# LuletterSoul/RP-Style-Transfer

Measured on AMD Instinct MI355X. Metric: stylized images/sec at 512×512, 1/2/4/8 MI355X; % HBM roofline, higher is better.
Workload: dtype fp32

## Files before the change

rp-style-transfer_amd/csrc/rpst_wino4.hip:

```cpp
#include "rpst_conv.h"
#include "rpst_wct.h"

#include <type_traits>

namespace rpst {

typedef __attribute__((address_space(3))) void* lds_ptr_t;

constexpr int kW4CK = 8;
#ifndef RPST_W4DBG
#define RPST_W4DBG 0
#endif
constexpr int kW4HW = 0, kW4HP = 2;
constexpr int kW4Ahead = 2, kW4Ahead2 = 3;
constexpr int kW4BM = 32;
constexpr int kW4TH = 16, kW4TW = 64;
constexpr int kW4PH = kW4TH + 2;
constexpr int kW4PS = 68;
constexpr int kW4CS = 1280;
constexpr int kW4DMA = 20;
constexpr int kW4DMA4 = 5;
constexpr int kW4WCH = 36 * kW4BM * kW4CK;
constexpr int kW4SPATCH = 4 * kW4CS;
constexpr int kW4SW = kW4WCH / 2;
// ... 127 lines not shown
  const float* btab;
  float2* statp;
};

__device__ __forceinline__ void bt6(float& d0, float& d1, float& d2, float& d3, float& d4,
                                    float& d5) {
  const float A = fmaf(-4.f, d2, d4), B = fmaf(-4.f, d1, d3);
  const float C = d4 - d2, E = d3 - d1;
  const float t0 = fmaf(4.f, d0, fmaf(-5.f, d2, d4));
  const float t5 = fmaf(4.f, d1, fmaf(-5.f, d3, d5));
  d0 = t0;
  d1 = A + B;
  d2 = A - B;
  d3 = fmaf(2.f, E, C);
  d4 = fmaf(-2.f, E, C);
  d5 = t5;
}

template <int NR, int INOP, bool STATS, bool BTAB, bool RELU>
__global__ __launch_bounds__(W4Geo<NR>::NTH, W4Geo<NR>::LAUNCH_WPE) void wino4_mfma_kernel(ConvArgs a) {
  using Geo = W4Geo<NR>;
  constexpr int S = Geo::STG, NW = Geo::NW, NH = Geo::NH;
  constexpr int DBG = RPST_W4DBG;
  static_assert(RawN<INOP>::R == 1, "one raw load per patch element");
  __shared__ __attribute__((aligned(16))) float smem0[Geo::STAGE];
  __shared__ __attribute__((aligned(16))) float smem1[Geo::STAGE];
  __shared__ __attribute__((aligned(16))) float smem2[S > 2 ? Geo::STAGE : 4];
  __shared__ __attribute__((aligned(16))) float smem3[S > 3 ? Geo::STAGE : 4];
  __shared__ __attribute__((aligned(16))) float dummy[256];

  int bid = (int)blockIdx.x;
  const int cog = bid % a.cosplit;
  bid /= a.cosplit;
  const int nct = a.co_tiles / a.cosplit;
  const int ct0 = cog * nct;
  int tx, ty, n;
  w4_tile(bid, a.tiles_x, a.tiles_y, tx, ty, n);
  const int nch = a.nchunks, K4 = 2 * nch, G = nct * K4;
  const int y0 = ty * Geo::TH, x0 = tx * kW4TW;

  const int tid = threadIdx.x;
  const int lane = tid & 63, wave = __builtin_amdgcn_readfirstlane(tid >> 6);
  const int k = lane >> 4, tn = lane & 15;
  const int wr = wave % NR, ph = wave / NR;

  const bool pooled = INOP == RPST_IN_UPSAMPLE2;
  const unsigned in_plane = pooled ? (unsigned)(a.Hs * a.Ws) : (unsigned)(a.H * a.W);
  const unsigned oob = a.Cin * in_plane * 4u;
  const float* in_img = conv_in_img(a, n, (int64_t)a.Cin * in_plane);
  const unsigned wbytes = (unsigned)(a.co_tiles * nch * kW4WCH) * 4u;
  const float* w_img = a.wpk + (int64_t)n * a.wstride;


  const int chl = wave / NH, hf = wave % NH;
  const bool zp = a.pad == RPST_PAD_ZERO;
  const int rs = pooled ? a.Ws : a.W;
  constexpr bool kAff = INOP == RPST_IN_ADAIN;
  constexpr int kSlow = Geo::SLOW, kWide = Geo::WIDE;
  unsigned poff[kSlow];
  unsigned pvalid = 0;
  const bool wide = !pooled && x0 >= 1 && x0 + kW4TW < a.W;
  {
    if (wide) {
#pragma unroll
      for (int i = 0; i < kWide; ++i) {
        const int p = kWide * hf + i;
        const int f = 64 * p + lane, row = min(f / 17, Geo::PH - 1), j = f - (f / 17) * 17;
        int y = y0 - 1 + row;
        const bool ok = p < Geo::DMA4 && f < Geo::PH * 17 && resolve_bf(y, a.H, zp);
        poff[i] = ok ? ((unsigned)(y * rs) + (unsigned)(x0 - 1 + 4 * j)) * 4u : oob;
        pvalid |= ok ? (1u << i) : 0u;
      }
    } else {
#pragma unroll
      for (int i = 0; i < kSlow; ++i) {
        const int f = 64 * (kSlow * hf + i) + lane;
        const int row = min(f / kW4PS, Geo::PH - 1), col = f - (f / kW4PS) * kW4PS;
        int y = y0 - 1 + row, x = x0 - 1 + col;
        const bool oky = resolve_bf(y, a.H, zp), okx = resolve_bf(x, a.W, zp);
        const bool ok = col < kW4TW + 2 && oky && okx;
        poff[i] = ok ? ((unsigned)((pooled ? y >> 1 : y) * rs) + (unsigned)(pooled ? x >> 1 : x)) * 4u
                     : oob;
        pvalid |= ok ? (1u << i) : 0u;
      }
    }
  }
  __shared__ float aparm[kAff ? 3 * kW4AffC : 1];
  if constexpr (kAff) {
    for (int c = tid; c < a.Cin; c += Geo::NTH) {
      const AdainP p = adain_params(a.aux, n, c, a);
      aparm[c] = p.mc;
      aparm[kW4AffC + c] = p.scale;
      aparm[2 * kW4AffC + c] = p.ms;
    }
    __syncthreads();
  }
  floatx4 acc[18][2];
#pragma unroll
  for (int x = 0; x < 18; ++x) acc[x][0] = acc[x][1] = floatx4{0.f, 0.f, 0.f, 0.f};

  auto issue_w = [&](int g, bool live, float* st) {
    if (!(DBG & 2)) {
      constexpr int WC = Geo::WPI - 1, REST = 18 - WC * NW;
      static_assert(REST > 0 && REST <= NW, "one remainder piece per wave at the most");
      const int wv = launder(wave);
      const int sw = ((ct0 * K4 + g) * kW4SW + wv * (WC * 256)) * 4;
      const auto r = rsrc_or_zero(w_img, wbytes, live);
      float* t = st + Geo::SPATCH + wv * (WC * 256);
      static_assert(WC == 2 || WC == 4, "the contiguous pieces below");
      __builtin_amdgcn_raw_ptr_buffer_load_lds(r, (lds_ptr_t)t, 16, lane * 16, sw, 0, 0);
      __builtin_amdgcn_raw_ptr_buffer_load_lds(r, (lds_ptr_t)t, 16, lane * 16, sw, 1024, 0);
      if constexpr (WC == 4) {
        __builtin_amdgcn_raw_ptr_buffer_load_lds(r, (lds_ptr_t)t, 16, lane * 16, sw, 2048, 0);
        __builtin_amdgcn_raw_ptr_buffer_load_lds(r, (lds_ptr_t)t, 16, lane * 16, sw, 3072, 0);
      }
      const bool real = wv < REST;
      __builtin_amdgcn_raw_ptr_buffer_load_lds(
          rsrc_or_zero(w_img, wbytes, live && real),
          (lds_ptr_t)(real ? st + Geo::SPATCH + (WC * NW + wv) * 256 : dummy), 16, lane * 16,
          sw + (WC * NW - (WC - 1) * wv) * 1024, 0, 0);
    }
  };
  auto issue_p = [&](int ks, bool live, float* st) {
    {
      if (DBG & 1) return;
      const int wv = launder(wave);
      const int c = 4 * ks + wv / NH;
      const bool ok = live && c < a.Cin;
      const auto r = rsrc_or_zero(in_img, oob, ok);
      const int so = ok ? (int)((unsigned)c * in_plane * 4u) : 0;
      float* xs = st + (wv / NH) * Geo::CS;
      if (wide) {
#pragma unroll
        for (int i = 0; i < kWide; ++i) {
          const int p = kWide * (wv % NH) + i;
          __builtin_amdgcn_raw_ptr_buffer_load_lds(
              r, (lds_ptr_t)(p < Geo::DMA4 ? xs + 256 * p : dummy), 16, (int)poff[i], so, 0, 0);
        }
      } else {
#pragma unroll
        for (int i = 0; i < kSlow; ++i)
          __builtin_amdgcn_raw_ptr_buffer_load_lds(r, (lds_ptr_t)(xs + 64 * (kSlow * (wv % NH) + i)),
                                                   4, (int)poff[i], so, 0, 0);
      }
    }
  };
  [[maybe_unused]] auto issue = [&](int g, int ks, bool live, float* st) {
    issue_w(g, live, st);
    issue_p(ks, live, st);
  };
  auto fix_own = [&](int g, float* st) {
    if constexpr (kAff) {
      if (DBG & 4) return;
      const int ks = g % K4, ch = 4 * ks + chl;
      const bool chok = ch < a.Cin;
      const int cc = chok ? ch : 0;
      const float mc = aparm[cc], sc = aparm[kW4AffC + cc], ms = aparm[2 * kW4AffC + cc];
      float* xs = st + chl * Geo::CS;
      if (wide) {
#pragma unroll
        for (int i = 0; i < kWide; ++i) {
          const int p = kWide * hf + i;
          if (p < Geo::DMA4) {
            float4* e = reinterpret_cast<float4*>(xs + 4 * (64 * p + lane));
            const bool ok = chok && ((pvalid >> i) & 1u);
            const float4 v = *e;
            *e = make_float4(ok ? fmaf(v.x - mc, sc, ms) : 0.f, ok ? fmaf(v.y - mc, sc, ms) : 0.f,
                             ok ? fmaf(v.z - mc, sc, ms) : 0.f, ok ? fmaf(v.w - mc, sc, ms) : 0.f);
          }
        }
      } else {
#pragma unroll
        for (int i = 0; i < kSlow; ++i) {
          float* e = xs + 64 * (kSlow * hf + i) + lane;
          const bool ok = chok && ((pvalid >> i) & 1u);
          *e = ok ? fmaf(*e - mc, sc, ms) : 0.f;
        }
      }
    }
  };


  auto load_rows = [&](const float* pbuf, float (&d)[5][6]) {
    const float* pr = pbuf + k * Geo::CS + (4 * wr + ph) * kW4PS + 4 * tn;
#pragma unroll
    for (int r = 0; r < 5; ++r) {
      floatx4 u = *reinterpret_cast<const floatx4*>(pr + r * kW4PS);
      floatx4 v = *reinterpret_cast<const floatx4*>(pr + r * kW4PS + 4);
      asm("" : "+v"(u), "+v"(v));
      d[r][0] = u[0];
      d[r][1] = u[1];
      d[r][2] = u[2];
      d[r][3] = u[3];
      d[r][4] = v[0];
      d[r][5] = v[1];
    }
  };
  auto compute = [&](const float* pbuf, float (&d)[5][6], auto&& hw, auto&& hp) {
    {
      const float* wq = pbuf + Geo::SPATCH + ph * 9 * 256 + lane * 4;
      float4 w4[9];
      constexpr int kA = NR == 4 ? kW4Ahead : kW4Ahead2;
#pragma unroll
      for (int q = 0; q < kA; ++q)
        w4[q] = (DBG & 64) ? make_float4(1.f, 2.f, 3.f, (float)q)
                           : *reinterpret_cast<const float4*>(wq + q * 256);
      float t[3][6];
      if (DBG & 8) {
#pragma unroll
        for (int i = 0; i < 3; ++i)
#pragma unroll
          for (int c = 0; c < 6; ++c) t[i][c] = d[i][c];
      } else if (ph == 0) {
#pragma unroll
        for (int c = 0; c < 6; ++c) {
          const float A = fmaf(-4.f, d[2][c], d[4][c]), B = fmaf(-4.f, d[1][c], d[3][c]);
          t[0][c] = fmaf(4.f, d[0][c], fmaf(-5.f, d[2][c], d[4][c]));
          t[1][c] = A + B;
          t[2][c] = A - B;
        }
      } else {
#pragma unroll
        for (int c = 0; c < 6; ++c) {
          const float C = d[3][c] - d[1][c], E = d[2][c] - d[0][c];
          t[0][c] = fmaf(2.f, E, C);
          t[1][c] = fmaf(-2.f, E, C);
          t[2][c] = fmaf(4.f, d[0][c], fmaf(-5.f, d[2][c], d[4][c]));
        }
      }
#pragma unroll
      for (int i = 0; i < 3; ++i)
        if (!(DBG & 8)) bt6(t[i][0], t[i][1], t[i][2], t[i][3], t[i][4], t[i][5]);
#pragma unroll
      for (int q = 0; q < 9; ++q) {
        if (q + kA < 9)
          w4[q + kA] = (DBG & 64) ? make_float4(1.f, 2.f, 3.f, (float)q)
                                  : *reinterpret_cast<const float4*>(wq + (q + kA) * 256);
        const int p0 = 2 * q, p1 = 2 * q + 1;
        const float v0 = t[p0 / 6][p0 % 6], v1 = t[p1 / 6][p1 % 6];
        acc[p0][0] = __builtin_amdgcn_mfma_f32_16x16x4f32(w4[q].x, v0, acc[p0][0], 0, 0, 0);
        acc[p0][1] = __builtin_amdgcn_mfma_f32_16x16x4f32(w4[q].y, v0, acc[p0][1], 0, 0, 0);
        acc[p1][0] = __builtin_amdgcn_mfma_f32_16x16x4f32(w4[q].z, v1, acc[p1][0], 0, 0, 0);
        acc[p1][1] = __builtin_amdgcn_mfma_f32_16x16x4f32(w4[q].w, v1, acc[p1][1], 0, 0, 0);
        if (q == kW4HW) hw();
        if (q == kW4HP) hp();
      }
    }
  };

  auto partial = [&](auto PHc, int mt, int r, float (&Y)[16], float b) {
    constexpr int PH = decltype(PHc)::value;
    float P[3][4];
#pragma unroll
    for (int i = 0; i < 3; ++i) {
      float m[6];
#pragma unroll
      for (int jj = 0; jj < 6; ++jj) m[jj] = acc[6 * i + jj][mt][r];
      at6(m, P[i]);
    }
    if constexpr (PH == 0) {
#pragma unroll
      for (int x = 0; x < 4; ++x) P[1][x] += b;
    }
#pragma unroll
    for (int x = 0; x < 4; ++x) {
      if constexpr (PH == 0) {
        const float s12 = P[1][x] + P[2][x], d12 = P[1][x] - P[2][x];
        Y[0 * 4 + x] = P[0][x] + s12;
        Y[1 * 4 + x] = d12;
        Y[2 * 4 + x] = s12;
        Y[3 * 4 + x] = d12;
      } else {
        const float s34 = P[0][x] + P[1][x], d34 = P[0][x] - P[1][x];
        Y[0 * 4 + x] = s34;
        Y[1 * 4 + x] = 2.f * d34;
        Y[2 * 4 + x] = 4.f * s34;
        Y[3 * 4 + x] = fmaf(8.f, d34, P[2][x]);
      }
    }
  };

  auto epi_ctx = [&]() {
    const KArgs L = late_args();
    EpiCtx e;
    e.W = L->W;
    e.H = L->H;
    e.Cout = L->Cout;
    e.slope = L->relu == RPST_ACT_RELU ? 0.f : (L->relu == RPST_ACT_LRELU ? 0.2f : 1.f);
    int btx, bty;
    w4_tile((int)blockIdx.x / L->cosplit, L->tiles_x, L->tiles_y, btx, bty, e.n);
    const int bx0 = btx * kW4TW;
    e.gy0 = bty * Geo::TH + 4 * wr;
    e.gx0 = bx0 + 4 * tn;
    e.vec = (e.W & 3) == 0 && e.gx0 + 3 < e.W;
    e.rows = max(0, min(4, e.H - e.gy0));
    const int cols = max(0, min(kW4TW, e.W - bx0));
// ... 145 lines not shown
    float bias8[2][4] = {{0.f, 0.f, 0.f, 0.f}, {0.f, 0.f, 0.f, 0.f}};
    if constexpr (PH == 0) {
      const float* bias = BTAB ? nullptr : late_args()->bias;
#pragma unroll
      for (int h = 0; h < 2; ++h)
#pragma unroll
        for (int r = 0; r < 4; ++r) {
          const int co = ct * kW4BM + 16 * h + 4 * k + r;
          if (co < e.Cout)
            bias8[h][r] = BTAB ? e.btab[((int64_t)e.n * e.Cout + co) * 9 + 4] : (bias ? bias[co] : 0.f);
        }
    }
#pragma unroll
    for (int r = 0; r < 4; ++r) {
      float own[16];
      {
        float give[16];
        partial(PHc, PH, r, own, bias8[0][r]);
        partial(PHc, 1 - PH, r, give, bias8[1][r]);
#pragma unroll
        for (int g4 = 0; g4 < 4; ++g4)
          *reinterpret_cast<float4*>(xb + ((PH * 4 + g4) * 64 + lane) * 4) =
              make_float4(give[4 * g4], give[4 * g4 + 1], give[4 * g4 + 2], give[4 * g4 + 3]);
      }
      lds_barrier();
#pragma unroll
      for (int g4 = 0; g4 < 4; ++g4) {
        const float4 o4 =
            *reinterpret_cast<const float4*>(xb + (((1 - PH) * 4 + g4) * 64 + lane) * 4);
        own[4 * g4] += o4.x;
        own[4 * g4 + 1] += o4.y;
        own[4 * g4 + 2] += o4.z;
        own[4 * g4 + 3] += o4.w;
      }
      finish(e, co0 + r, own);
      if (r < 3) lds_barrier();
    }
  };
  auto epilogue = [&](int ct, float* xs) {
    if (ph) epilogue_ph(std::integral_constant<int, 1>{}, ct, xs);
    else epilogue_ph(std::integral_constant<int, 0>{}, ct, xs);
  };

  auto wait_ahead2 = [&]() {
    if (DBG & 128) return;
    if constexpr (S == 2) {
      asm volatile("s_waitcnt vmcnt(0)" ::: "memory");
    } else {
      static_assert(S == 4 && Geo::WPI == 3 && kWide == 3 && kSlow == 10, "counted waits");
      if (wide) asm volatile("s_waitcnt vmcnt(12)" ::: "memory");
      else asm volatile("s_waitcnt vmcnt(26)" ::: "memory");
    }
  };
  issue(0, 0, true, smem0);
  if constexpr (S == 4) {
    issue(1, 1 % K4, G > 1, smem1);
    issue(2, 2 % K4, G > 2, smem2);
  }
  int ks3 = (S - 1) % K4;
  int ks = 0, ct = ct0;
  if constexpr (kAff) {
    wait_ahead2();
    fix_own(0, smem0);
  }
  auto step = [&](int g, float* cur, float* nx1, float* nx3) {
    wait_ahead2();
    lds_barrier();
    float d[5][6];
    load_rows(cur, d);
    const bool live3 = g + S - 1 < G;
    auto hw = [&]() { issue_w(g + S - 1, live3, nx3); };
    auto hp = [&]() { issue_p(ks3, live3, nx3); };
    compute(cur, d, hw, hp);
    ks3 = ks3 + 1 == K4 ? 0 : ks3 + 1;
    if (ks == K4 - 1) {
      if (!(DBG & 32)) epilogue(ct, cur);
#pragma unroll
      for (int x = 0; x < 18; ++x) acc[x][0] = acc[x][1] = floatx4{0.f, 0.f, 0.f, 0.f};
    }
    if constexpr (kAff) {
      if (g + 1 < G) {
        wait_ahead2();
        fix_own(g + 1, nx1);
      }
    }
    ct += ks == K4 - 1 ? 1 : 0;
    ks = ks == K4 - 1 ? 0 : ks + 1;
  };
  if constexpr (S == 4) {
    for (int g = 0; g < G; g += 4) {
      step(g, smem0, smem1, smem3);
      if (g + 1 < G) step(g + 1, smem1, smem2, smem0);
      if (g + 2 < G) step(g + 2, smem2, smem3, smem1);
      if (g + 3 < G) step(g + 3, smem3, smem0, smem2);
    }
  } else {
    for (int g = 0; g < G; g += 2) {
      step(g, smem0, smem1, smem1);
      if (g + 1 < G) step(g + 1, smem1, smem0, smem0);
    }
  }
  asm volatile("s_waitcnt vmcnt(0)" ::: "memory");
}

size_t wino4_fold_floats(int N, int Cin, int Cout) {
  return (size_t)N * (wino4_image_floats_max(Cout, Cin) + (size_t)Cout * 9) +
         2 * (size_t)9 * Cout * Cin + 2;
}

__global__ void wino4_fold_w_kernel(const float4* __restrict__ pk, float4* __restrict__ out,
                                    const float* __restrict__ aux, int N, int Cin, int nch,
                                    int64_t per4) {
  const int64_t t = (int64_t)blockIdx.x * blockDim.x + threadIdx.x;
  if (t >= (int64_t)N * per4) return;
  const int n = (int)(t / per4);
  const int64_t u = t - (int64_t)n * per4;
  const int l = (int)(u & 63);
  int64_t r = (u >> 6) / 9;
  const int s = (int)((r >> 1) & 1);
  const int c = (int)((r >> 2) % nch);
  const int ci = c * kW4CK + 4 * s + (l >> 4);
  const int64_t nc = (int64_t)N * Cin, i = (int64_t)n * Cin + (ci < Cin ? ci : 0);
  const float sc = ci < Cin ? aux[3 * nc + i] / aux[2 * nc + i] : 0.f;
  const float4 v = pk[u];
  out[t] = make_float4(v.x * sc, v.y * sc, v.z * sc, v.w * sc);
}

__global__ void class_sums_kernel(const float* __restrict__ dpk, double* __restrict__ S, int Cin,
                                  int Cout, int cout_pad, int reflect) {
  const int64_t t = (int64_t)blockIdx.x * blockDim.x + threadIdx.x;
  if (t >= (int64_t)9 * Cout * Cin) return;
  const int ci = (int)(t % Cin);
// ... 187 lines not shown
```

rp-style-transfer_amd/csrc/rpst_wino4q.hip:

```cpp
#include "rpst_conv.h"

#include <type_traits>

#ifndef RPST_W4Q_DBG
#define RPST_W4Q_DBG 0
#endif

namespace rpst {
namespace {

template <int PAD>
__device__ __forceinline__ void q_mfma(floatx4& acc, float a, float b) {
  if constexpr (PAD)
    asm volatile("s_nop 1\n\tv_mfma_f32_16x16x4_f32 %0, %1, %2, %0" : "+v"(acc) : "v"(a), "v"(b));
  else
    asm volatile("v_mfma_f32_16x16x4_f32 %0, %1, %2, %0" : "+v"(acc) : "v"(a), "v"(b));
}
__device__ __forceinline__ unsigned q_lds_addr(const float* p) {
  return (unsigned)(uintptr_t)(const __attribute__((address_space(3))) float*)p;
}
template <int OFF>
__device__ __forceinline__ void q_dma16(__amdgpu_buffer_rsrc_t r, unsigned m0, unsigned voff,
                                        int soff) {
  asm volatile("s_mov_b32 m0, %0\n\ts_nop 0\n\tbuffer_load_dwordx4 %1, %2, %3 offen offset:%4 lds"
               :: "s"(m0), "v"(voff), "s"(r), "s"(soff), "i"(OFF) : "memory");
}
__device__ __forceinline__ void q_dma4(__amdgpu_buffer_rsrc_t r, unsigned m0, unsigned voff,
                                       int soff) {
  asm volatile("s_mov_b32 m0, %0\n\ts_nop 0\n\tbuffer_load_dword %1, %2, %3 offen lds"
               :: "s"(m0), "v"(voff), "s"(r), "s"(soff) : "memory");
}
__device__ __forceinline__ int q_lane_here() {
  int z = 0;
#if __HIP_DEVICE_COMPILE__
  asm volatile("" : "+v"(z));
#endif
  return (int)__builtin_amdgcn_mbcnt_hi(~0u, __builtin_amdgcn_mbcnt_lo(~0u, (unsigned)z));
}
__device__ __forceinline__ void q_lds_barrier() {
  asm volatile("s_waitcnt lgkmcnt(0)" ::: "memory");
  __builtin_amdgcn_s_barrier();
}

template <int H>
__device__ __forceinline__ void q_bt3(float d0, float d1, float d2, float d3, float d4, float d5,
                                      float& u0, float& u1, float& u2) {
  if constexpr (H == 0) {
    const float A = fmaf(-4.f, d2, d4), B = fmaf(-4.f, d1, d3);
    u0 = fmaf(4.f, d0, fmaf(-5.f, d2, d4));
    u1 = A + B;
    u2 = A - B;
  } else {
    const float C = d4 - d2, E = d3 - d1;
    u0 = fmaf(2.f, E, C);
    u1 = fmaf(-2.f, E, C);
    u2 = fmaf(4.f, d1, fmaf(-5.f, d3, d5));
  }
}

}

constexpr int kQCo = 64;
constexpr int kQTH = 8, kQTW = 64;
constexpr int kQXO = 4;
constexpr int kQPS = 72;
constexpr int kQCS = 768;
constexpr int kQWS = 9216;
constexpr int kQPAT = 4 * kQCS;
constexpr int kQNTH = 512;
// ... 290 lines not shown
          for (int xx = 0; xx < 4; ++xx)
            if (gx0 + xx < W) o[yy * W + xx] = Y[yy * 4 + xx];
        }
      }
    }
  }
  if constexpr (STATS) {
    sum = row16_sum(sum);
    const float mean = sum * r.inv;
    float m2 = 0.f;
    if (full) {
#pragma unroll
      for (int i = 0; i < 16; ++i) m2 = fmaf(Y[i] - mean, Y[i] - mean, m2);
    } else {
      const int rows = r.rows, gx0 = r.bx0 + 4 * tn, W = r.W;
#pragma unroll
      for (int yy = 0; yy < 4; ++yy)
#pragma unroll
        for (int xx = 0; xx < 4; ++xx) {
          const float dv = Y[yy * 4 + xx] - mean;
          m2 += (yy < rows && gx0 + xx < W) ? dv * dv : 0.f;
        }
    }
    m2 = row16_sum(m2);
    if (tn == 0 && cok) ((gfloatx2*)r.stat)[co] = floatx2{mean, m2};
  }
}

template <int INOP, bool STATS, bool BTAB, bool RELU>
__global__ __launch_bounds__(kQNTH, 1) void wino4q_mfma_kernel(ConvArgs a) {
  __shared__ __attribute__((aligned(16))) float ws0[kQWS];
  __shared__ __attribute__((aligned(16))) float ws1[kQWS];
  __shared__ __attribute__((aligned(16))) float ps0[kQPAT];
  __shared__ __attribute__((aligned(16))) float ps1[kQPAT];
  __shared__ __attribute__((aligned(16))) float ps2[kQPAT];
  __shared__ __attribute__((aligned(16))) float ps3[kQPAT];
  __shared__ __attribute__((aligned(16))) float dummy[256];
  __shared__ unsigned poffs[kQSlow][kQNTH];
  __shared__ float btl[BTAB ? 9 * kQMaxCo : kQMaxCo];

  const int wave = __builtin_amdgcn_readfirstlane((int)threadIdx.x >> 6);
  int lane = threadIdx.x & 63;
  const int wr = wave >> 2;

  int bid = (int)blockIdx.x;
  const int cog = bid % a.cosplit;
  bid /= a.cosplit;
  const int nct = a.co_tiles / a.cosplit, ct0 = cog * nct;
  int tx, ty, n;
  w4_tile(bid, a.tiles_x, a.tiles_y, tx, ty, n);
  const int K4 = a.nchunks, G = nct * K4;
  const int y0 = ty * kQTH, x0 = tx * kQTW;

  {
    const int nb = BTAB ? 9 * a.Cout : a.Cout;
    const float* src = BTAB ? a.btab + (int64_t)n * nb : a.bias;
    for (int i = threadIdx.x; i < nb; i += kQNTH) btl[i] = src ? src[i] : 0.f;
  }
  __shared__ __attribute__((aligned(16))) QEpiRec erec[2];
  __shared__ uint4 evoff[2 * 16];
  if (threadIdx.x < 32) q_epi_fill(a, tx, ty, n, (int)threadIdx.x, erec, evoff);
  constexpr bool up = INOP == RPST_IN_UPSAMPLE2;
  const unsigned in_plane = up ? (unsigned)(a.Hs * a.Ws) : (unsigned)(a.H * a.W);
  const unsigned oob = a.Cin * in_plane * 4u;
  const float* in_img = conv_in_img(a, n, (int64_t)a.Cin * in_plane);
  const unsigned wbytes = (unsigned)(nct * K4 * kQWS) * 4u;
  const float* w_img = a.wpk + (int64_t)n * a.wstride + (int64_t)ct0 * K4 * kQWS;

  const int hf = wave & 1;
  const bool zp = a.pad == RPST_PAD_ZERO;
  const int rs = up ? a.Ws : a.W;
  const bool w4a = (a.W & 3) == 0;
  const bool wide = !up && ((x0 >= 1 && x0 + kQTW < a.W) || (w4a && x0 + kQTW <= a.W));
  const bool fixL = wide && w4a && !zp && x0 == 0;
  const bool fixR = wide && w4a && !zp && x0 + kQTW == a.W;
  unsigned poff[kQSlow];
  int tid = threadIdx.x;
  if (wide) {
#pragma unroll
    for (int i = 0; i < kQWide; ++i) {
      const int p = kQWide * hf + i;
      const int f = 64 * p + lane, row = min(f / kQRP, 9), j = f - (f / kQRP) * kQRP;
      int y = y0 - 1 + row;
      const int xs = x0 - kQXO + 4 * j;
      const bool okx = !w4a || (xs >= 0 && xs + 3 < a.W);
      const bool ok = p < kQDMA4 && f < 10 * kQRP && resolve_bf(y, a.H, zp) && okx;
      poff[i] = ok ? ((unsigned)(y * rs) + (unsigned)xs) * 4u : oob;
    }
#pragma unroll
    for (int i = kQWide; i < kQSlow; ++i) poff[i] = oob;
  } else {
#pragma unroll
    for (int i = 0; i < kQSlow; ++i) {
      const int p = kQSlow * hf + i;
      const int f = 64 * p + lane;
      const int row = min(f / kQPS, 9), col = f - (f / kQPS) * kQPS;
      int y = y0 - 1 + row, x = x0 - kQXO + col;
      const bool oky = resolve_bf(y, a.H, zp), okx = resolve_bf(x, a.W, zp);
      const bool ok = p < kQDMA && col >= kQXO - 1 && col < kQXO + 1 + kQTW &&
                      f < 10 * kQPS && oky && okx;
      poff[i] = ok ? ((unsigned)((up ? y >> 1 : y) * rs) + (unsigned)(up ? x >> 1 : x)) * 4u : oob;
    }
  }
#pragma unroll
  for (int i = 0; i < kQSlow; ++i) poffs[i][tid] = poff[i];

  constexpr int DBG = RPST_W4Q_DBG;
  const int wl = wave * 4096;
  const bool real4 = wave < 4;
  const int w4 = 32768 + wave * 1024;
  const unsigned dummy_a = q_lds_addr(dummy);
  int wso = wl;
  auto issue_w = [&](bool live, unsigned stg, auto Ic) {
    constexpr int I = decltype(Ic)::value;
    if (DBG & 2) return;
    if constexpr (I < 4) {
      q_dma16<1024 * I>(rsrc_or_zero(w_img, wbytes, live), stg + wl, lane * 16, wso);
    } else {
      q_dma16<0>(rsrc_or_zero(w_img, wbytes, live && real4), real4 ? stg + w4 : dummy_a,
                 lane * 16, wso + (w4 - wl));
    }
  };
  const unsigned pstep = 4u * in_plane * 4u;
  const int pbase = (int)((unsigned)(wave >> 1) * in_plane * 4u);
  const bool h1 = (wave & 1) != 0;
  const int pl = (wave >> 1) * (kQCS * 4) + (h1 ? (wide ? 2048 : kQSlow * 256) : 0);
  int pso = pbase;
  auto issue_p = [&](auto WIDEc, bool live, unsigned stg) {
    constexpr bool WIDE = decltype(WIDEc)::value;
    if (DBG & 1) return;
    const auto r = rsrc_or_zero(in_img, oob, live);
    const unsigned xs = stg + launder(pl);
    if constexpr (WIDE) {
      q_dma16<0>(r, xs, poffs[0][tid], pso);
      q_dma16<0>(r, h1 ? dummy_a : xs + 1024, poffs[1][tid], pso);
    } else {
#pragma unroll
      for (int i = 0; i < kQSlow; ++i) q_dma4(r, xs + 256 * i, poffs[i][tid], pso);
    }
    pso += (int)pstep;
  };
  const bool bst_all = !a.pool_out && (a.W & 3) == 0 &&
                       (int64_t)a.Cout * a.H * a.W * 4 < (1LL << 31);
  bool post_epi = false;
  auto wait_ring = [&](bool first) {
    if (DBG & 128) return;
    if (first && post_epi && bst_all) {
      if (wide) asm volatile("s_waitcnt vmcnt(18)" ::: "memory");
      else asm volatile("s_waitcnt vmcnt(22)" ::: "memory");
    } else if (wide) {
      asm volatile("s_waitcnt vmcnt(2)" ::: "memory");
    } else {
      asm volatile("s_waitcnt vmcnt(6)" ::: "memory");
    }
    if (first) post_epi = false;
  };

  auto fix_halo = [&](float* stg) {
    if ((wave == 0 && fixL) || (wave == 1 && fixR)) {
      const int l = q_lane_here();
      if (l < 40) {
        const int ch = l / 10, row = l - 10 * ch;
        float* rp = stg + ch * kQCS + row * kQPS;
        if (wave == 0) rp[kQXO - 1] = rp[kQXO + 1];
        else rp[kQXO + kQTW] = rp[kQXO + kQTW - 2];
      }
    }
  };
  auto prologue = [&](auto WIDEc) {
    issue_p(WIDEc, true, q_lds_addr(ps0));
    issue_p(WIDEc, true, q_lds_addr(ps1));
    issue_w(true, q_lds_addr(ws0), std::integral_constant<int, 0>{});
    issue_w(true, q_lds_addr(ws0), std::integral_constant<int, 1>{});
    issue_w(true, q_lds_addr(ws0), std::integral_constant<int, 2>{});
    issue_w(true, q_lds_addr(ws0), std::integral_constant<int, 3>{});
    issue_w(true, q_lds_addr(ws0), std::integral_constant<int, 4>{});
    issue_p(WIDEc, true, q_lds_addr(ps2));
    issue_p(WIDEc, true, q_lds_addr(ps3));
  };
  if (wide) prologue(std::true_type{});
  else prologue(std::false_type{});
  wait_ring(false);
  q_lds_barrier();
  if (fixL || fixR) {
    fix_halo(ps0);
    fix_halo(ps1);
    q_lds_barrier();
  }

  auto body = [&](auto Qc) {
    constexpr int Q = decltype(Qc)::value, QR = Q >> 1, QC = Q & 1;
    lane = q_lane_here();
    tid = wave * 64 + lane;
    const int k = lane >> 4, tn = lane & 15;
    floatx4 acc[9][4];
#pragma unroll
    for (int p = 0; p < 9; ++p)
#pragma unroll
      for (int cb = 0; cb < 4; ++cb) acc[p][cb] = floatx4{0.f, 0.f, 0.f, 0.f};
    const int roff = k * kQCS + (4 * wr + QR) * kQPS + 4 * tn;
    auto read_row = [&](const float* stg, int rr, float (&d)[8]) {
      const float* rp = stg + roff + rr * kQPS;
      floatx4 u = *reinterpret_cast<const floatx4*>(rp + 4);
      const float e = QC ? rp[8] : rp[3];
      asm("" : "+v"(u));
      d[0] = QC ? 0.f : e; d[1] = u[0]; d[2] = u[1]; d[3] = u[2]; d[4] = u[3];
      d[5] = QC ? e : 0.f; d[6] = 0.f; d[7] = 0.f;
    };
    auto col_pass = [&](const float (&d)[8], float (&u)[3]) {
      if (DBG & 8) {
        u[0] = d[0]; u[1] = d[1]; u[2] = d[2];
        return;
      }
      q_bt3<QC>(d[0], d[1], d[2], d[3], d[4], d[5], u[0], u[1], u[2]);
    };
    auto row_pass = [&](const float (&u)[5][3], int j, float (&v)[9]) {
      if (DBG & 8) {
        v[j] = u[0][j]; v[3 + j] = u[2][j]; v[6 + j] = u[4][j];
        return;
      }
      if constexpr (QR == 0)
        q_bt3<0>(u[0][j], u[1][j], u[2][j], u[3][j], u[4][j], 0.f, v[j], v[3 + j], v[6 + j]);
      else
        q_bt3<1>(0.f, u[0][j], u[1][j], u[2][j], u[3][j], u[4][j], v[j], v[3 + j], v[6 + j]);
    };
    float V[9];
    {
      float u[5][3];
#pragma unroll
      for (int rr = 0; rr < 5; ++rr) {
        float d[8];
        read_row(ps0, rr, d);
        col_pass(d, u[rr]);
      }
#pragma unroll
      for (int j = 0; j < 3; ++j) row_pass(u, j, V);
    }

    const int woff = Q * 9 * 256 + lane * 4;
    int x = 0;
    auto step = [&](float* wsx, float* psn, float* wsn, float* psx, float* pfx, int ks,
                    bool first) {
      wait_ring(first);
      const bool wlive = x + 1 < G, plive = x + 4 < G;
      wso += kQWS * 4;
      if (first && ks + 4 == K4) pso = pbase;
      const unsigned wsn_a = q_lds_addr(wsn), psx_a = q_lds_addr(psx);
      if (DBG & 16) asm volatile("s_waitcnt lgkmcnt(0)" ::: "memory");
      else q_lds_barrier();
      constexpr int ord[9] = {0, 3, 6, 1, 4, 7, 2, 5, 8};
      constexpr int kA = kQAhead;
      float4 w4[9];
#pragma unroll
      for (int q = 0; q < kA; ++q)
        w4[ord[q]] = *reinterpret_cast<const float4*>(wsx + woff + ord[q] * 256);
      float d[8];
      read_row(psn, 0, d);
      float u[5][3];
#pragma unroll
      for (int q = 0; q < 9; ++q) {
        const int p = ord[q];
        if (q + kA < 9)
          w4[ord[q + kA]] = *reinterpret_cast<const float4*>(wsx + woff + ord[q + kA] * 256);
        q_mfma<1>(acc[p][0], w4[p].x, V[p]);
        q_mfma<0>(acc[p][1], w4[p].y, V[p]);
        q_mfma<0>(acc[p][2], w4[p].z, V[p]);
        q_mfma<0>(acc[p][3], w4[p].w, V[p]);
        if (q == kQWG0) issue_w(wlive, wsn_a, std::integral_constant<int, 0>{});
        if (q == kQWG0 + 1) issue_w(wlive, wsn_a, std::integral_constant<int, 1>{});
        if (q == kQWG0 + 2) issue_w(wlive, wsn_a, std::integral_constant<int, 2>{});
        if (q == kQWG0 + 3) issue_w(wlive, wsn_a, std::integral_constant<int, 3>{});
        if (q == kQWG0 + 4) issue_w(wlive, wsn_a, std::integral_constant<int, 4>{});
        if (q == kQPG) {
          if (wide) issue_p(std::true_type{}, plive, psx_a);
          else issue_p(std::false_type{}, plive, psx_a);
        }
        if (q < 5) {
          col_pass(d, u[q]);
          if (q + 1 < 5) read_row(psn, q + 1, d);
        }
        if (q == 5 || q == 6 || q == 8) row_pass(u, q == 8 ? 2 : q - 5, V);
        if (q == 7) fix_halo(pfx);
      }
      ++x;
    };

    auto epilogue = [&](int ctile) {
      if (DBG & 32) {
        float t = 0.f;
#pragma unroll
        for (int p = 0; p < 9; ++p)
#pragma unroll
          for (int cb = 0; cb < 4; ++cb) t += acc[p][cb][0];
        if (t == 1.2345f) late_args()->out[threadIdx.x] = t;
#pragma unroll
        for (int p = 0; p < 9; ++p)
#pragma unroll
          for (int cb = 0; cb < 4; ++cb) acc[p][cb] = floatx4{0.f, 0.f, 0.f, 0.f};
        return;
      }
      q_lds_barrier();
      asm volatile("s_nop 7\n\ts_nop 4" : "+v"(acc[0][0]), "+v"(acc[0][1]), "+v"(acc[0][2]),
                   "+v"(acc[0][3]), "+v"(acc[1][0]), "+v"(acc[1][1]), "+v"(acc[1][2]),
                   "+v"(acc[1][3]), "+v"(acc[2][0]), "+v"(acc[2][1]), "+v"(acc[2][2]),
                   "+v"(acc[2][3]), "+v"(acc[3][0]), "+v"(acc[3][1]), "+v"(acc[3][2]),
                   "+v"(acc[3][3]), "+v"(acc[4][0]), "+v"(acc[4][1]));
      asm volatile("" : "+v"(acc[4][2]), "+v"(acc[4][3]), "+v"(acc[5][0]), "+v"(acc[5][1]),
                   "+v"(acc[5][2]), "+v"(acc[5][3]), "+v"(acc[6][0]), "+v"(acc[6][1]),
                   "+v"(acc[6][2]), "+v"(acc[6][3]), "+v"(acc[7][0]), "+v"(acc[7][1]),
                   "+v"(acc[7][2]), "+v"(acc[7][3]), "+v"(acc[8][0]), "+v"(acc[8][1]),
                   "+v"(acc[8][2]), "+v"(acc[8][3]));
      const int el = q_lane_here(), ek = el >> 4, etn = el & 15;
      const int co0 = ctile * kQCo + 16 * Q + 4 * ek;
      unsigned cofs = (unsigned)co0 * erec[wr].hw4;
      asm volatile("" : "+v"(cofs));
#pragma unroll
      for (int rp = 0; rp < 2; ++rp) {
        float P[2][6][4];
#pragma unroll
        for (int pt = 0; pt < 3; ++pt) {
          float* xb = ws1 + wr * kQXS;
#pragma unroll
          for (int dq = 0; dq < 4; ++dq) {
            if (dq == Q || (DBG & 4)) continue;
            const int slot = (Q - dq - 1) & 3;
#pragma unroll
            for (int j = 0; j < 3; ++j)
              *reinterpret_cast<float2*>(xb + (((dq * 3 + slot) * 3 + j) * 64 + el) * 2) =
                  make_float2(acc[3 * pt + j][dq][2 * rp], acc[3 * pt + j][dq][2 * rp + 1]);
          }
          if (!(DBG & 4)) q_lds_barrier();
          float m[2][2][6];
#pragma unroll
          for (int s = 0; s < 4; ++s) {
#pragma unroll
            for (int j = 0; j < 3; ++j) {
              float2 v;
              if (s == Q || (DBG & 4)) {
                const int src = (DBG & 4) ? s : Q;
                v = make_float2(acc[3 * pt + j][src][2 * rp], acc[3 * pt + j][src][2 * rp + 1]);
              } else {
                v = *reinterpret_cast<const float2*>(
                    xb + (((Q * 3 + ((s - Q - 1) & 3)) * 3 + j) * 64 + el) * 2);
              }
              m[0][s >> 1][3 * (s & 1) + j] = v.x;
              m[1][s >> 1][3 * (s & 1) + j] = v.y;
            }
          }
#pragma unroll
          for (int e2 = 0; e2 < 2; ++e2) {
            at6(m[e2][0], P[e2][pt]);
            at6(m[e2][1], P[e2][3 + pt]);
          }
          if (!(DBG & 4) && (rp == 0 || pt < 2)) q_lds_barrier();
        }
#pragma unroll
        for (int e2 = 0; e2 < 2; ++e2) {
          const int r = 2 * rp + e2;
          float bias = 0.f;
          {
            const int co = co0 + r;
            if (co < erec[wr].Cout) bias = BTAB ? btl[co * 9 + 4] : btl[co];
          }
#pragma unroll
          for (int x = 0; x < 4; ++x) P[e2][1][x] += bias;
          float Y[16];
#pragma unroll
          for (int x = 0; x < 4; ++x) {
            float c6[6], y[4];
#pragma unroll
            for (int I = 0; I < 6; ++I) c6[I] = P[e2][I][x];
            at6(c6, y);
#pragma unroll
            for (int yy = 0; yy < 4; ++yy) Y[yy * 4 + x] = y[yy];
          }
          q_finish<STATS, BTAB, RELU>(erec[wr], evoff[wr * 16 + etn], btl, co0 + r, cofs, Y, etn);
          cofs += erec[wr].hw4;
        }
      }
#pragma unroll
      for (int p = 0; p < 9; ++p)
#pragma unroll
        for (int cb = 0; cb < 4; ++cb) acc[p][cb] = floatx4{0.f, 0.f, 0.f, 0.f};
    };

    int ks = 0, ct = ct0;
    for (int g = 0; g < G; g += 4) {
      step(ws0, ps1, ws1, ps0, ps2, ks, true);
      step(ws1, ps2, ws0, ps1, ps3, ks + 1, false);
      step(ws0, ps3, ws1, ps2, ps0, ks + 2, false);
      step(ws1, ps0, ws0, ps3, ps1, ks + 3, false);
      ks += 4;
      if (ks == K4) {
        epilogue(ct);
        post_epi = true;
        ks = 0;
        ++ct;
      }
    }
  };
  switch (wave & 3) {
    case 0: body(std::integral_constant<int, 0>{}); break;
    case 1: body(std::integral_constant<int, 1>{}); break;
    case 2: body(std::integral_constant<int, 2>{}); break;
    default: body(std::integral_constant<int, 3>{}); break;
  }
  asm volatile("s_waitcnt vmcnt(0)" ::: "memory");
}

int wino4q_launch(ConvArgs& a, int in_op, hipStream_t st) {
  RPST_REQUIRE(in_op == RPST_IN_NONE || in_op == RPST_IN_UPSAMPLE2,
               "conv2d: winograd4 (quarter) does not support in_op %d", in_op);
  const ConvTiling t = wino4q_tiling(a);
  RPST_REQUIRE((int64_t)a.co_tiles * a.nchunks * kQWS * 4 < (1LL << 31),
               "conv2d: winograd4 weight image exceeds 2 GiB");
  RPST_REQUIRE(t.blocks <= 0x7fffffffLL, "conv2d: grid too large");
  const unsigned nb = (unsigned)t.blocks;
  const bool stats = a.stat_part != nullptr, btab = a.btab != nullptr;
  RPST_REQUIRE(!btab || in_op == RPST_IN_NONE, "conv2d: winograd4 bias table with a loader op");
  RPST_REQUIRE(!(stats && btab), "conv2d: winograd4 folded bias with statistics");
#define RPST_W4Q_GO(OP, S, B)                                                  \
  do {                                                                         \
    if (a.relu == RPST_ACT_RELU)                                               \
      wino4q_mfma_kernel<OP, S, B, true><<<nb, kQNTH, 0, st>>>(a);             \
    else                                                                       \
      wino4q_mfma_kernel<OP, S, B, false><<<nb, kQNTH, 0, st>>>(a);            \
  } while (0)
  if (in_op == RPST_IN_UPSAMPLE2) {
    if (stats) RPST_W4Q_GO(RPST_IN_UPSAMPLE2, true, false);
    else RPST_W4Q_GO(RPST_IN_UPSAMPLE2, false, false);
  } else {
    if (stats) RPST_W4Q_GO(RPST_IN_NONE, true, false);
    else if (btab) RPST_W4Q_GO(RPST_IN_NONE, false, true);
    else RPST_W4Q_GO(RPST_IN_NONE, false, false);
  }
#undef RPST_W4Q_GO
  return launch_status("wino4q_mfma_kernel");
}

}
```

Before: 582.0.

## Zero accumulators via MFMA zero-C and issue DMA before setup work

The first MFMA of each output tile now takes a zero C operand instead of the accumulator, so the explicit accumulator zeroing after each epilogue and at kernel start is removed. The first weight and patch DMAs are issued earlier: before offset and affine setup in wino4, and before bias-table, epilogue-record and offset-spill stores in wino4q, using register offsets for the prologue. This hides global load latency behind setup work and frees VALU slots. The wino4q main loop is restructured into per-tile turns, which assumes K4 is a multiple of 4.

```diff
diff --git a/rp-style-transfer_amd/csrc/rpst_wino4.hip b/rp-style-transfer_amd/csrc/rpst_wino4.hip
--- a/rp-style-transfer_amd/csrc/rpst_wino4.hip
+++ b/rp-style-transfer_amd/csrc/rpst_wino4.hip
@@ -203,53 +203,6 @@
   const float* w_img = a.wpk + (int64_t)n * a.wstride;
 
 
-  const int chl = wave / NH, hf = wave % NH;
-  const bool zp = a.pad == RPST_PAD_ZERO;
-  const int rs = pooled ? a.Ws : a.W;
-  constexpr bool kAff = INOP == RPST_IN_ADAIN;
-  constexpr int kSlow = Geo::SLOW, kWide = Geo::WIDE;
-  unsigned poff[kSlow];
-  unsigned pvalid = 0;
-  const bool wide = !pooled && x0 >= 1 && x0 + kW4TW < a.W;
-  {
-    if (wide) {
-#pragma unroll
-      for (int i = 0; i < kWide; ++i) {
-        const int p = kWide * hf + i;
-        const int f = 64 * p + lane, row = min(f / 17, Geo::PH - 1), j = f - (f / 17) * 17;
-        int y = y0 - 1 + row;
-        const bool ok = p < Geo::DMA4 && f < Geo::PH * 17 && resolve_bf(y, a.H, zp);
-        poff[i] = ok ? ((unsigned)(y * rs) + (unsigned)(x0 - 1 + 4 * j)) * 4u : oob;
-        pvalid |= ok ? (1u << i) : 0u;
-      }
-    } else {
-#pragma unroll
-      for (int i = 0; i < kSlow; ++i) {
-        const int f = 64 * (kSlow * hf + i) + lane;
-        const int row = min(f / kW4PS, Geo::PH - 1), col = f - (f / kW4PS) * kW4PS;
-        int y = y0 - 1 + row, x = x0 - 1 + col;
-        const bool oky = resolve_bf(y, a.H, zp), okx = resolve_bf(x, a.W, zp);
-        const bool ok = col < kW4TW + 2 && oky && okx;
-        poff[i] = ok ? ((unsigned)((pooled ? y >> 1 : y) * rs) + (unsigned)(pooled ? x >> 1 : x)) * 4u
-                     : oob;
-        pvalid |= ok ? (1u << i) : 0u;
-      }
-    }
-  }
-  __shared__ float aparm[kAff ? 3 * kW4AffC : 1];
-  if constexpr (kAff) {
-    for (int c = tid; c < a.Cin; c += Geo::NTH) {
-      const AdainP p = adain_params(a.aux, n, c, a);
-      aparm[c] = p.mc;
-      aparm[kW4AffC + c] = p.scale;
-      aparm[2 * kW4AffC + c] = p.ms;
-    }
-    __syncthreads();
-  }
-  floatx4 acc[18][2];
-#pragma unroll
-  for (int x = 0; x < 18; ++x) acc[x][0] = acc[x][1] = floatx4{0.f, 0.f, 0.f, 0.f};
-
   auto issue_w = [&](int g, bool live, float* st) {
     if (!(DBG & 2)) {
       constexpr int WC = Geo::WPI - 1, REST = 18 - WC * NW;
@@ -272,6 +225,53 @@
           sw + (WC * NW - (WC - 1) * wv) * 1024, 0, 0);
     }
   };
+  issue_w(0, true, smem0);
+
+  const int chl = wave / NH, hf = wave % NH;
+  const bool zp = a.pad == RPST_PAD_ZERO;
+  const int rs = pooled ? a.Ws : a.W;
+  constexpr bool kAff = INOP == RPST_IN_ADAIN;
+  constexpr int kSlow = Geo::SLOW, kWide = Geo::WIDE;
+  unsigned poff[kSlow];
+  unsigned pvalid = 0;
+  const bool wide = !pooled && x0 >= 1 && x0 + kW4TW < a.W;
+  {
+    if (wide) {
+#pragma unroll
+      for (int i = 0; i < kWide; ++i) {
+        const int p = kWide * hf + i;
+        const int f = 64 * p + lane, row = min(f / 17, Geo::PH - 1), j = f - (f / 17) * 17;
+        int y = y0 - 1 + row;
+        const bool ok = p < Geo::DMA4 && f < Geo::PH * 17 && resolve_bf(y, a.H, zp);
+        poff[i] = ok ? ((unsigned)(y * rs) + (unsigned)(x0 - 1 + 4 * j)) * 4u : oob;
+        pvalid |= ok ? (1u << i) : 0u;
+      }
+    } else {
+#pragma unroll
+      for (int i = 0; i < kSlow; ++i) {
+        const int f = 64 * (kSlow * hf + i) + lane;
+        const int row = min(f / kW4PS, Geo::PH - 1), col = f - (f / kW4PS) * kW4PS;
+        int y = y0 - 1 + row, x = x0 - 1 + col;
+        const bool oky = resolve_bf(y, a.H, zp), okx = resolve_bf(x, a.W, zp);
+        const bool ok = col < kW4TW + 2 && oky && okx;
+        poff[i] = ok ? ((unsigned)((pooled ? y >> 1 : y) * rs) + (unsigned)(pooled ? x >> 1 : x)) * 4u
+                     : oob;
+        pvalid |= ok ? (1u << i) : 0u;
+      }
+    }
+  }
+  __shared__ float aparm[kAff ? 3 * kW4AffC : 1];
+  if constexpr (kAff) {
+    for (int c = tid; c < a.Cin; c += Geo::NTH) {
+      const AdainP p = adain_params(a.aux, n, c, a);
+      aparm[c] = p.mc;
+      aparm[kW4AffC + c] = p.scale;
+      aparm[2 * kW4AffC + c] = p.ms;
+    }
+    __syncthreads();
+  }
+  floatx4 acc[18][2];
+
   auto issue_p = [&](int ks, bool live, float* st) {
     {
       if (DBG & 1) return;
@@ -347,8 +347,10 @@
       d[r][5] = v[1];
     }
   };
-  auto compute = [&](const float* pbuf, float (&d)[5][6], auto&& hw, auto&& hp) {
+  auto compute = [&](auto SETc, const float* pbuf, float (&d)[5][6], auto&& hw, auto&& hp) {
     {
+      constexpr bool SET = decltype(SETc)::value;
+      constexpr floatx4 kZero = {0.f, 0.f, 0.f, 0.f};
       const float* wq = pbuf + Geo::SPATCH + ph * 9 * 256 + lane * 4;
       float4 w4[9];
       constexpr int kA = NR == 4 ? kW4Ahead : kW4Ahead2;
@@ -389,10 +391,10 @@
                                   : *reinterpret_cast<const float4*>(wq + (q + kA) * 256);
         const int p0 = 2 * q, p1 = 2 * q + 1;
         const float v0 = t[p0 / 6][p0 % 6], v1 = t[p1 / 6][p1 % 6];
-        acc[p0][0] = __builtin_amdgcn_mfma_f32_16x16x4f32(w4[q].x, v0, acc[p0][0], 0, 0, 0);
-        acc[p0][1] = __builtin_amdgcn_mfma_f32_16x16x4f32(w4[q].y, v0, acc[p0][1], 0, 0, 0);
-        acc[p1][0] = __builtin_amdgcn_mfma_f32_16x16x4f32(w4[q].z, v1, acc[p1][0], 0, 0, 0);
-        acc[p1][1] = __builtin_amdgcn_mfma_f32_16x16x4f32(w4[q].w, v1, acc[p1][1], 0, 0, 0);
+        acc[p0][0] = __builtin_amdgcn_mfma_f32_16x16x4f32(w4[q].x, v0, SET ? kZero : acc[p0][0], 0, 0, 0);
+        acc[p0][1] = __builtin_amdgcn_mfma_f32_16x16x4f32(w4[q].y, v0, SET ? kZero : acc[p0][1], 0, 0, 0);
+        acc[p1][0] = __builtin_amdgcn_mfma_f32_16x16x4f32(w4[q].z, v1, SET ? kZero : acc[p1][0], 0, 0, 0);
+        acc[p1][1] = __builtin_amdgcn_mfma_f32_16x16x4f32(w4[q].w, v1, SET ? kZero : acc[p1][1], 0, 0, 0);
         if (q == kW4HW) hw();
         if (q == kW4HP) hp();
       }
@@ -644,7 +646,7 @@
       else asm volatile("s_waitcnt vmcnt(26)" ::: "memory");
     }
   };
-  issue(0, 0, true, smem0);
+  issue_p(0, true, smem0);
   if constexpr (S == 4) {
     issue(1, 1 % K4, G > 1, smem1);
     issue(2, 2 % K4, G > 2, smem2);
@@ -663,13 +665,10 @@
     const bool live3 = g + S - 1 < G;
     auto hw = [&]() { issue_w(g + S - 1, live3, nx3); };
     auto hp = [&]() { issue_p(ks3, live3, nx3); };
-    compute(cur, d, hw, hp);
+    if (ks == 0) compute(std::true_type{}, cur, d, hw, hp);
+    else compute(std::false_type{}, cur, d, hw, hp);
     ks3 = ks3 + 1 == K4 ? 0 : ks3 + 1;
-    if (ks == K4 - 1) {
-      if (!(DBG & 32)) epilogue(ct, cur);
-#pragma unroll
-      for (int x = 0; x < 18; ++x) acc[x][0] = acc[x][1] = floatx4{0.f, 0.f, 0.f, 0.f};
-    }
+    if (ks == K4 - 1 && !(DBG & 32)) epilogue(ct, cur);
     if constexpr (kAff) {
       if (g + 1 < G) {
         wait_ahead2();
diff --git a/rp-style-transfer_amd/csrc/rpst_wino4q.hip b/rp-style-transfer_amd/csrc/rpst_wino4q.hip
--- a/rp-style-transfer_amd/csrc/rpst_wino4q.hip
+++ b/rp-style-transfer_amd/csrc/rpst_wino4q.hip
@@ -15,6 +15,13 @@
     asm volatile("s_nop 1\n\tv_mfma_f32_16x16x4_f32 %0, %1, %2, %0" : "+v"(acc) : "v"(a), "v"(b));
   else
     asm volatile("v_mfma_f32_16x16x4_f32 %0, %1, %2, %0" : "+v"(acc) : "v"(a), "v"(b));
+}
+template <int PAD>
+__device__ __forceinline__ void q_mfma_set(floatx4& acc, float a, float b) {
+  if constexpr (PAD)
+    asm volatile("s_nop 1\n\tv_mfma_f32_16x16x4_f32 %0, %1, %2, 0" : "=&v"(acc) : "v"(a), "v"(b));
+  else
+    asm volatile("v_mfma_f32_16x16x4_f32 %0, %1, %2, 0" : "=&v"(acc) : "v"(a), "v"(b));
 }
 __device__ __forceinline__ unsigned q_lds_addr(const float* p) {
   return (unsigned)(uintptr_t)(const __attribute__((address_space(3))) float*)p;
@@ -411,14 +418,8 @@
   const int K4 = a.nchunks, G = nct * K4;
   const int y0 = ty * kQTH, x0 = tx * kQTW;
 
-  {
-    const int nb = BTAB ? 9 * a.Cout : a.Cout;
-    const float* src = BTAB ? a.btab + (int64_t)n * nb : a.bias;
-    for (int i = threadIdx.x; i < nb; i += kQNTH) btl[i] = src ? src[i] : 0.f;
-  }
   __shared__ __attribute__((aligned(16))) QEpiRec erec[2];
   __shared__ uint4 evoff[2 * 16];
-  if (threadIdx.x < 32) q_epi_fill(a, tx, ty, n, (int)threadIdx.x, erec, evoff);
   constexpr bool up = INOP == RPST_IN_UPSAMPLE2;
   const unsigned in_plane = up ? (unsigned)(a.Hs * a.Ws) : (unsigned)(a.H * a.W);
   const unsigned oob = a.Cin * in_plane * 4u;
@@ -461,8 +462,6 @@
       poff[i] = ok ? ((unsigned)((up ? y >> 1 : y) * rs) + (unsigned)(up ? x >> 1 : x)) * 4u : oob;
     }
   }
-#pragma unroll
-  for (int i = 0; i < kQSlow; ++i) poffs[i][tid] = poff[i];
 
   constexpr int DBG = RPST_W4Q_DBG;
   const int wl = wave * 4096;
@@ -485,17 +484,18 @@
   const bool h1 = (wave & 1) != 0;
   const int pl = (wave >> 1) * (kQCS * 4) + (h1 ? (wide ? 2048 : kQSlow * 256) : 0);
   int pso = pbase;
-  auto issue_p = [&](auto WIDEc, bool live, unsigned stg) {
-    constexpr bool WIDE = decltype(WIDEc)::value;
+  auto issue_p = [&](auto WIDEc, bool live, unsigned stg, auto REGc) {
+    constexpr bool WIDE = decltype(WIDEc)::value, REG = decltype(REGc)::value;
     if (DBG & 1) return;
     const auto r = rsrc_or_zero(in_img, oob, live);
     const unsigned xs = stg + launder(pl);
     if constexpr (WIDE) {
-      q_dma16<0>(r, xs, poffs[0][tid], pso);
-      q_dma16<0>(r, h1 ? dummy_a : xs + 1024, poffs[1][tid], pso);
+      q_dma16<0>(r, xs, REG ? poff[0] : poffs[0][tid], pso);
+      q_dma16<0>(r, h1 ? dummy_a : xs + 1024, REG ? poff[1] : poffs[1][tid], pso);
     } else {
 #pragma unroll
-      for (int i = 0; i < kQSlow; ++i) q_dma4(r, xs + 256 * i, poffs[i][tid], pso);
+      for (int i = 0; i < kQSlow; ++i)
+        q_dma4(r, xs + 256 * i, REG ? poff[i] : poffs[i][tid], pso);
     }
     pso += (int)pstep;
   };
@@ -527,18 +527,26 @@
     }
   };
   auto prologue = [&](auto WIDEc) {
-    issue_p(WIDEc, true, q_lds_addr(ps0));
-    issue_p(WIDEc, true, q_lds_addr(ps1));
+    issue_p(WIDEc, true, q_lds_addr(ps0), std::true_type{});
+    issue_p(WIDEc, true, q_lds_addr(ps1), std::true_type{});
     issue_w(true, q_lds_addr(ws0), std::integral_constant<int, 0>{});
     issue_w(true, q_lds_addr(ws0), std::integral_constant<int, 1>{});
     issue_w(true, q_lds_addr(ws0), std::integral_constant<int, 2>{});
     issue_w(true, q_lds_addr(ws0), std::integral_constant<int, 3>{});
     issue_w(true, q_lds_addr(ws0), std::integral_constant<int, 4>{});
-    issue_p(WIDEc, true, q_lds_addr(ps2));
-    issue_p(WIDEc, true, q_lds_addr(ps3));
+    issue_p(WIDEc, true, q_lds_addr(ps2), std::true_type{});
+    issue_p(WIDEc, true, q_lds_addr(ps3), std::true_type{});
   };
   if (wide) prologue(std::true_type{});
   else prologue(std::false_type{});
+#pragma unroll
+  for (int i = 0; i < kQSlow; ++i) poffs[i][tid] = poff[i];
+  {
+    const int nb = BTAB ? 9 * a.Cout : a.Cout;
+    const float* src = BTAB ? a.btab + (int64_t)n * nb : a.bias;
+    for (int i = threadIdx.x; i < nb; i += kQNTH) btl[i] = src ? src[i] : 0.f;
+  }
+  if (threadIdx.x < 32) q_epi_fill(a, tx, ty, n, (int)threadIdx.x, erec, evoff);
   wait_ring(false);
   q_lds_barrier();
   if (fixL || fixR) {
@@ -553,10 +561,13 @@
     tid = wave * 64 + lane;
     const int k = lane >> 4, tn = lane & 15;
     floatx4 acc[9][4];
-#pragma unroll
-    for (int p = 0; p < 9; ++p)
-#pragma unroll
-      for (int cb = 0; cb < 4; ++cb) acc[p][cb] = floatx4{0.f, 0.f, 0.f, 0.f};
+    auto acc_open = [&]() {
+#pragma unroll
+      for (int p = 0; p < 9; ++p)
+#pragma unroll
+        for (int cb = 0; cb < 4; ++cb) asm volatile("" : "=v"(acc[p][cb]));
+    };
+    acc_open();
     const int roff = k * kQCS + (4 * wr + QR) * kQPS + 4 * tn;
     auto read_row = [&](const float* stg, int rr, float (&d)[8]) {
       const float* rp = stg + roff + rr * kQPS;
@@ -598,8 +609,9 @@
 
     const int woff = Q * 9 * 256 + lane * 4;
     int x = 0;
-    auto step = [&](float* wsx, float* psn, float* wsn, float* psx, float* pfx, int ks,
-                    bool first) {
+    auto step = [&](auto SETc, float* wsx, float* psn, float* wsn, float* psx, float* pfx,
+                    int ks, bool first) {
+      constexpr bool SET = decltype(SETc)::value;
       wait_ring(first);
       const bool wlive = x + 1 < G, plive = x + 4 < G;
       wso += kQWS * 4;
@@ -621,18 +633,25 @@
         const int p = ord[q];
         if (q + kA < 9)
           w4[ord[q + kA]] = *reinterpret_cast<const float4*>(wsx + woff + ord[q + kA] * 256);
-        q_mfma<1>(acc[p][0], w4[p].x, V[p]);
-        q_mfma<0>(acc[p][1], w4[p].y, V[p]);
-        q_mfma<0>(acc[p][2], w4[p].z, V[p]);
-        q_mfma<0>(acc[p][3], w4[p].w, V[p]);
+        if constexpr (SET) {
+          q_mfma_set<1>(acc[p][0], w4[p].x, V[p]);
+          q_mfma_set<0>(acc[p][1], w4[p].y, V[p]);
+          q_mfma_set<0>(acc[p][2], w4[p].z, V[p]);
+          q_mfma_set<0>(acc[p][3], w4[p].w, V[p]);
+        } else {
+          q_mfma<1>(acc[p][0], w4[p].x, V[p]);
+          q_mfma<0>(acc[p][1], w4[p].y, V[p]);
+          q_mfma<0>(acc[p][2], w4[p].z, V[p]);
+          q_mfma<0>(acc[p][3], w4[p].w, V[p]);
+        }
         if (q == kQWG0) issue_w(wlive, wsn_a, std::integral_constant<int, 0>{});
         if (q == kQWG0 + 1) issue_w(wlive, wsn_a, std::integral_constant<int, 1>{});
         if (q == kQWG0 + 2) issue_w(wlive, wsn_a, std::integral_constant<int, 2>{});
         if (q == kQWG0 + 3) issue_w(wlive, wsn_a, std::integral_constant<int, 3>{});
         if (q == kQWG0 + 4) issue_w(wlive, wsn_a, std::integral_constant<int, 4>{});
         if (q == kQPG) {
-          if (wide) issue_p(std::true_type{}, plive, psx_a);
-          else issue_p(std::false_type{}, plive, psx_a);
+          if (wide) issue_p(std::true_type{}, plive, psx_a, std::false_type{});
+          else issue_p(std::false_type{}, plive, psx_a, std::false_type{});
         }
         if (q < 5) {
           col_pass(d, u[q]);
@@ -737,25 +756,22 @@
           cofs += erec[wr].hw4;
         }
       }
-#pragma unroll
-      for (int p = 0; p < 9; ++p)
-#pragma unroll
-        for (int cb = 0; cb < 4; ++cb) acc[p][cb] = floatx4{0.f, 0.f, 0.f, 0.f};
+      acc_open();
     };
 
-    int ks = 0, ct = ct0;
-    for (int g = 0; g < G; g += 4) {
-      step(ws0, ps1, ws1, ps0, ps2, ks, true);
-      step(ws1, ps2, ws0, ps1, ps3, ks + 1, false);
-      step(ws0, ps3, ws1, ps2, ps0, ks + 2, false);
-      step(ws1, ps0, ws0, ps3, ps1, ks + 3, false);
-      ks += 4;
-      if (ks == K4) {
-        epilogue(ct);
-        post_epi = true;
-        ks = 0;
-        ++ct;
-      }
+    auto turn = [&](auto SETc, int ks) {
+      step(SETc, ws0, ps1, ws1, ps0, ps2, ks, true);
+      step(std::false_type{}, ws1, ps2, ws0, ps1, ps3, ks + 1, false);
+      step(std::false_type{}, ws0, ps3, ws1, ps2, ps0, ks + 2, false);
+      step(std::false_type{}, ws1, ps0, ws0, ps3, ps1, ks + 3, false);
+    };
+    int ct = ct0;
+    for (int g = 0; g < G; g += K4) {
+      turn(std::true_type{}, 0);
+      for (int ks = 4; ks < K4; ks += 4) turn(std::false_type{}, ks);
+      epilogue(ct);
+      post_epi = true;
+      ++ct;
     }
   };
   switch (wave & 3) {
```

After: 585.8 (median of 6 runs). Within noise of the previous version (+0.7%).
